# TimoLassmann/kalign

Hardware: AMD Instinct MI355X
Metric: GCUPS (DP cell updates/s) on NxL synthetic MSA (higher is better)
Workload: dtype f32

## Files before the change

kalign_amd/csrc/ka_meetup.h:

```cpp
#pragma once

struct KaLevelOut { int2* items; int* prog; int* nitems; int2* pack16; int2* pack4; int* n16; int* n4; int* nsub; int* rowalloc; int srows;
                    int sub_ok, kind, nres, sub_bytes; };
#define KA_ITEM_SUBTREE 2
#define KA_SUB_MARK 0x7fffffff

__device__ __forceinline__ bool ka_child_is_subtree(const KaLevelOut& o, int rows, int cols)
{
        return o.sub_ok && rows <= KA_SUB_MAXROWS && ka_sub_bytes(o.kind, o.nres, rows, cols) <= o.sub_bytes && cols < 4096;
}

#if KA_TP
#define KA_LONG_COLS 40
#else
#define KA_LONG_COLS 96
#endif
__device__ __forceinline__ bool ka_pass_is_strip(int nrows, int ncols) { return nrows > 32 || (nrows > 2 && ncols >= KA_LONG_COLS); }

__device__ __forceinline__ void ka_emit_pass(const KaLevelOut& o, int slot, int dir, int nrows, int ncols)
{
        if (ka_pass_is_strip(nrows, ncols)) {
                const int ns = ka_strips_of(nrows, o.srows);
                const int base = atomicAdd(o.nitems, ns);
                for (int k = 0; k < ns; ++k) { o.items[base + k] = make_int2(slot, (dir << 16) | k); o.prog[base + k] = 0; }
        } else if (nrows > 8) {
                o.pack16[atomicAdd(o.n16, 1)] = make_int2(slot, dir);
        } else {
                o.pack4[atomicAdd(o.n4, 1)] = make_int2(slot, dir);
        }
}

__device__ __forceinline__ void ka_emit_items(const KaLevelOut& o, int slot, int starta, int enda, int ncols, bool allow_sub = true)
{
        if (allow_sub && ka_child_is_subtree(o, enda - starta, ncols)) {
                const int base = atomicAdd(o.nitems, 1);
                o.items[base] = make_int2(slot, KA_ITEM_SUBTREE << 16); o.prog[base] = 0;
                return;
        }
        const int mid = ((enda - starta) / 2) + starta;
        ka_emit_pass(o, slot, KA_FWD, mid - starta, ncols);
        ka_emit_pass(o, slot, KA_BWD, enda - mid, ncols);
}

__device__ __forceinline__ int ka_level_srows(const TaskShared& S, int level)
{
        if (!S.q1_lvl) return S.srows;
        if (S.split || level > 12) return KA_STRIP_ROWS;
        const int pr = (S.La + (2 << level) - 1) >> (level + 1);
        const long long strips = (long long)(2 << level) * ((pr + KA_STRIP1_ROWS - 1) / KA_STRIP1_ROWS);
        return strips <= 4ll * S.G ? KA_STRIP1_ROWS : KA_STRIP_ROWS;
}

__device__ __forceinline__ KaLevelOut ka_level_out(TaskShared& S, int parity, bool next)
{
        KaLevelOut o;
        o.items = S.items[parity]; o.prog = S.prog[parity];
        o.pack16 = S.pack[parity][0]; o.pack4 = S.pack[parity][1];
        (void)next;
        o.nitems = &S.lctl->lvl[parity].nitems;
        o.n16 = &S.lctl->lvl[parity].npack[0];
        o.n4 = &S.lctl->lvl[parity].npack[1];
        o.nsub = &S.lctl->lvl[parity].nsub;
        o.rowalloc = &S.lctl->lvl[parity].rowalloc;
        o.srows = S.lvl_srows[parity];
        o.sub_ok = S.sub_ok; o.kind = S.kind; o.nres = S.nres_t; o.sub_bytes = S.sub_stride;
        return o;
}

template <int KIND, int GL, bool FLIP = false, bool REC = false, bool MW = false, bool RU = false>
__device__ __forceinline__ void ka_meetup(TaskShared& S, const KaSub* qc, const int k0, const int ncur, KaSub* qnext,
                                          const KaLevelOut& lout, const int wlane, const bool top_level, const int kdig = 0, const int lvl = 0)
{
        static_assert(!MW || GL == 64, "the multi-wave scan works on 64-lane groups");
        const int lane = wlane % GL;
        const int ksub = k0 + wlane / GL;
        const bool in_range = ksub < ncur;
        const KaSub sb = qc[in_range ? ksub : k0];
        const bool rec = REC || S.rec_on;
        const bool valid = in_range && (FLIP || rec || sb.pad != KA_SUB_MARK);
        const bool is_top = top_level && ksub == 0;
        const int startb = sb.startb, endb = sb.endb;
        const int mid = ((sb.enda - sb.starta) / 2) + sb.starta;
        const bool ru = RU && S.reuse_ok != 0;
        const bool f_taken = ru && sb.fsrc >= 0, b_taken = ru && sb.bsrc >= 0;
        const KaState* f = f_taken ? S.sfbuf[(lvl + 1) & 1] + sb.fsrc : S.fbuf + sb.roff;
        const KaState* b = b_taken ? S.sbbuf[(lvl + 1) & 1] + sb.bsrc : S.bbuf + sb.roff;
        const float middle = (float)(endb - startb) / 2.0f + (float)startb;
        const int rrec = mid + 1;
        float g3, g7, g6n, g6f;
        if (KIND == KA_SS) {
                g3 = -S.gpo; g7 = -S.gpo;
                g6n = (startb == 0) ? -S.tgpe : -S.gpe;
                g6f = (endb == S.Lb) ? -S.tgpe : -S.gpe;
        } else {
                const float* R = S.p1 + ((long long)rrec << 6);
                g3 = R[55] * S.p1_mult; g7 = R[55 - 64] * S.p1_mult;
                g6n = (startb == 0) ? R[57] * S.p1_mult : R[56] * S.p1_mult;
                g6f = (endb == S.Lb) ? R[57] * S.p1_mult : R[56] * S.p1_mult;
        }
        Best B = { -KA_F, -KA_F, 0x7fffffff, 0x7fffffff };
        const int mw_wave = MW ? (int)(threadIdx.x >> 6) : 0, mw_nw = MW ? KA_NW : 1;
        for (int i = startb + lane + GL * mw_wave; valid && i <= endb; i += GL * mw_nw) {
                KaState fi = f[i - startb], bi = b[i - startb];
                if (RU) { if (b_taken && i == startb) bi.ga = -KA_F; if (f_taken && i == endb) fi.ga = -KA_F; }
                float sub = fabsf(middle - (float)i);
                sub = sub / 1000.0f;
                const int kb = (i - startb) * 8;
                if (i < endb) {
                        float c2, c5, dummy1, dummy2;
                        col_terms<KIND>(S, i + 1, c2, dummy1, dummy2);
                        col_terms<KIND>(S, i, c5, dummy1, dummy2);
                        best_consider(B, fi.a + bi.a - sub, kb + 0);
                        best_consider(B, fi.a + bi.ga + c2 - sub, kb + 1);
                        best_consider(B, fi.a + bi.gb + g3 - sub, kb + 2);
                        best_consider(B, fi.ga + bi.a + c5 - sub, kb + 3);
                        best_consider(B, fi.gb + bi.gb + g6n - sub, kb + 4);
                        best_consider(B, fi.gb + bi.a + g7 - sub, kb + 5);
                } else {
                        best_consider(B, fi.a + bi.gb + g3 - sub, kb + 2);
                        best_consider(B, fi.gb + bi.gb + g6f - sub, kb + 4);
                }
        }
#pragma unroll
        for (int off = GL / 2; off >= 1; off >>= 1) {
                const float omx = __shfl_xor(B.mx, off, 64);
                const float omx2 = __shfl_xor(B.mx2, off, 64);
                const int okey = __shfl_xor(B.key, off, 64);
                const int okey2 = FLIP ? __shfl_xor(B.key2, off, 64) : 0x7fffffff;
                best_merge(B, omx, omx2, okey, okey2);
        }
        if (MW) {
                if (lane == 0) { S.mw_mx[mw_wave] = B.mx; S.mw_mx2[mw_wave] = B.mx2; S.mw_key[mw_wave] = B.key; }
                __syncthreads();
                if (mw_wave != 0) return;
                B.mx = -KA_F; B.mx2 = -KA_F; B.key = 0x7fffffff; B.key2 = 0x7fffffff;
                for (int w = 0; w < mw_nw; ++w) best_merge(B, S.mw_mx[w], S.mw_mx2[w], S.mw_key[w]);
        }
        const bool leader = (lane == 0) && valid;
        int meet = -1, tr = -1;
        if (leader && B.key != 0x7fffffff) {
                const int ord = B.key & 7;
                meet = startb + (B.key >> 3);
                tr = ord + 1 + (ord >= 3 ? 1 : 0);
        }
        if (leader && is_top) { S.ctl->top_meet = meet; S.ctl->top_tr = tr; S.ctl->top_score = B.mx; }
        if (rec && leader && B.mx2 > -KA_F) {
                const int idx = atomicAdd(&S.ctl->nrec, 1);
                S.mrec[idx] = make_int2(sb.pad, __float_as_int(B.mx - B.mx2));
                if (REC && S.inc) { const KaInc I = ka_inc_view(S); I.win[idx] = sb; I.mx[idx] = make_int2(3 * kdig, S.raw[sb.starta]); }
        }
        if (FLIP && leader) {
                if (B.mx2 > -KA_F) { S.rf.msum += B.mx - B.mx2; S.rf.mcount += 1; }
                if (S.rf.thr > 0.0f && B.key2 != 0x7fffffff && B.mx2 > -KA_F) {
                        const float margin = B.mx - B.mx2;
                        if (margin < S.rf.thr) {
                                if (S.rf.trial > 0 && S.rf.counter % S.rf.stride == S.rf.trial - 1) {
                                        const int ord2 = B.key2 & 7;
                                        meet = startb + (B.key2 >> 3);
                                        tr = ord2 + 1 + (ord2 >= 3 ? 1 : 0);
                                }
                                S.rf.counter += 1;
                        }
                }
        }

        const KaState Z = { 0.0f, -KA_F, -KA_F };
        const KaState GA = { -KA_F, 0.0f, -KA_F };
        const KaState GB = { -KA_F, -KA_F, 0.0f };
        KaSub c1, c2;
        c1.starta = sb.starta; c1.startb = startb; c1.fin = sb.fin;
        c2.enda = sb.enda; c2.endb = endb; c2.bin = sb.bin;
        c1.enda = c1.starta; c1.endb = c1.startb; c1.bin = Z;
        c2.starta = c2.enda; c2.startb = c2.endb; c2.fin = Z;
        c1.pad = rec ? sb.pad + kdig : 0; c2.pad = rec ? sb.pad + 2 * kdig : 0; c1.roff = 0; c2.roff = 0;
        c1.fsrc = -1; c1.bsrc = -1; c2.fsrc = -1; c2.bsrc = -1;
        if (tr > 0) {
                int* path = S.raw;
                switch (tr) {
                case 1:
                        path[mid] = meet; path[mid + 1] = meet + 1;
                        c1.enda = mid - 1; c1.endb = meet - 1; c1.bin = Z;
                        c2.starta = mid + 1; c2.startb = meet + 1; c2.fin = Z;
                        break;
                case 2:
                        path[mid] = meet;
                        c1.enda = mid - 1; c1.endb = meet - 1; c1.bin = Z;
                        c2.starta = mid; c2.startb = meet + 1; c2.fin = GA;
                        break;
                case 3:
                        path[mid] = meet;
                        c1.enda = mid - 1; c1.endb = meet - 1; c1.bin = Z;
                        c2.starta = mid + 1; c2.startb = meet; c2.fin = GB;
                        break;
                case 5:
                        path[mid + 1] = meet + 1;
                        c1.enda = mid; c1.endb = meet - 1; c1.bin = GA;
                        c2.starta = mid + 1; c2.startb = meet + 1; c2.fin = Z;
                        break;
                case 6:
                        c1.enda = mid - 1; c1.endb = meet; c1.bin = GB;
                        c2.starta = mid + 1; c2.startb = meet; c2.fin = GB;
                        break;
                default:
                        path[mid + 1] = meet + 1;
                        c1.enda = mid - 1; c1.endb = meet; c1.bin = GB;
                        c2.starta = mid + 1; c2.startb = meet + 1; c2.fin = Z;
                        break;
                }
        }
        const bool v1 = (tr > 0) && c1.starta < c1.enda && c1.startb < c1.endb;
        const bool v2 = (tr > 0) && c2.starta < c2.enda && c2.startb < c2.endb;
        int need[5] = {0, 0, 0, 0, 0};
        int pr[4], pc[4];
        {
                const int m1 = ((c1.enda - c1.starta) / 2) + c1.starta, m2 = ((c2.enda - c2.starta) / 2) + c2.starta;
                pr[0] = m1 - c1.starta; pr[1] = c1.enda - m1; pr[2] = m2 - c2.starta; pr[3] = c2.enda - m2;
                pc[0] = pc[1] = c1.endb - c1.startb; pc[2] = pc[3] = c2.endb - c2.startb;
        }
        if (v1) { need[0] += 1; need[1] += c1.endb - c1.startb + 1; }
        if (v2) { need[0] += 1; need[1] += c2.endb - c2.startb + 1; }
        const bool st1 = !FLIP && !rec && v1 && ka_child_is_subtree(lout, c1.enda - c1.starta, c1.endb - c1.startb);
        const bool st2 = !FLIP && !rec && v2 && ka_child_is_subtree(lout, c2.enda - c2.starta, c2.endb - c2.startb);
        if (st1) need[2] += 1;
        if (st2) need[2] += 1;
        bool take_f1 = false, take_b2 = false;
        if (RU && ru && !FLIP && !rec) {
                const int nfp = mid - sb.starta, nbp = sb.enda - mid, pcols = endb - startb;
                const int rs_f = (nfp - 1) / 2, rs_b = nbp / 2;
                take_f1 = v1 && !st1 && !f_taken && rs_f >= 1 && ka_pass_is_strip(nfp, pcols) && pr[0] == rs_f;
                take_b2 = v2 && !st2 && !b_taken && rs_b >= 1 && ka_pass_is_strip(nbp, pcols) && pr[3] == rs_b;
                if (take_f1) c1.fsrc = sb.roff;
                if (take_b2) c2.bsrc = sb.roff + (c2.startb - startb);
        }
#pragma unroll
        for (int x = 0; x < 4; ++x) {
                if (!((x < 2) ? v1 : v2) || ((x < 2) ? st1 : st2)) continue;
                if (RU && ((x == 0 && take_f1) || (x == 3 && take_b2))) continue;
                if (ka_pass_is_strip(pr[x], pc[x])) need[2] += ka_strips_of(pr[x], lout.srows);
                else if (pr[x] > 8) need[3] += 1;
                else need[4] += 1;
        }
        float marg = 0.0f;
        int mc = 0;
        if (leader && B.mx2 > -KA_F) { marg = B.mx - B.mx2; mc = 1; }
        int off[5], tot[5];
#pragma unroll
        for (int x = 0; x < 5; ++x) {
                int sc = need[x];
#pragma unroll
                for (int d = 1; d < 64; d <<= 1) { const int y = __shfl_up(sc, d, 64); if (wlane >= d) sc += y; }
                tot[x] = __shfl(sc, 63, 64);
                off[x] = sc - need[x];
        }
        double msum_w = (double)marg;
        int mcnt_w = mc;
#pragma unroll
        for (int d = 32; d >= 1; d >>= 1) { msum_w += __shfl_xor(msum_w, d, 64); mcnt_w += __shfl_xor(mcnt_w, d, 64); }
        int base[5] = {0, 0, 0, 0, 0};
        if (wlane == 0) {
                if (tot[0]) base[0] = atomicAdd(lout.nsub, tot[0]);
                if (tot[1]) base[1] = atomicAdd(lout.rowalloc, tot[1]);
                if (tot[2]) base[2] = atomicAdd(lout.nitems, tot[2]);
                if (tot[3]) base[3] = atomicAdd(lout.n16, tot[3]);
                if (tot[4]) base[4] = atomicAdd(lout.n4, tot[4]);
                if (mcnt_w) { atomicAdd(&S.lctl->msum, msum_w); atomicAdd(&S.lctl->mcount, mcnt_w); }
        }
#pragma unroll
        for (int x = 0; x < 5; ++x) base[x] = __shfl(base[x], 0, 64) + off[x];
        if (!leader || tr < 0) return;
        int slot = base[0], row = base[1], ip = base[2], p16 = base[3], p4 = base[4];
#pragma unroll
        for (int ch = 0; ch < 2; ++ch) {
                KaSub& cs = ch ? c2 : c1;
                if (!(ch ? v2 : v1)) continue;
                cs.roff = row; row += cs.endb - cs.startb + 1;
                if (ch ? st2 : st1) cs.pad = KA_SUB_MARK;
                qnext[slot] = cs;
                if (ch ? st2 : st1) {
                        lout.items[ip] = make_int2(slot, KA_ITEM_SUBTREE << 16); lout.prog[ip] = 0; ++ip; ++slot;
                        continue;
                }
#pragma unroll
                for (int x = 0; x < 2; ++x) {
                        const int nrows = pr[2 * ch + x], ncols = pc[2 * ch + x], dir = x ? KA_BWD : KA_FWD;
                        if (RU && ((ch == 0 && x == 0 && take_f1) || (ch == 1 && x == 1 && take_b2))) continue;
                        if (ka_pass_is_strip(nrows, ncols)) {
                                const int ns = ka_strips_of(nrows, lout.srows);
                                for (int k = 0; k < ns; ++k) { lout.items[ip + k] = make_int2(slot, (dir << 16) | k); lout.prog[ip + k] = 0; }
                                ip += ns;
                        } else if (nrows > 8) {
                                lout.pack16[p16++] = make_int2(slot, dir);
                        } else {
                                lout.pack4[p4++] = make_int2(slot, dir);
                        }
                }
                ++slot;
        }
}
```

kalign_amd/csrc/ka_path.h:

```cpp
#pragma once

__device__ void ka_code_path(TaskShared& S, int* lds)
{
        const int tid = threadIdx.x;
        const int len_a = S.len_a, len_b = S.len_b;
        const int* raw = S.raw;
        if (S.swapped) {
                int* r2 = S.raw2;
                for (int i = tid; i < len_a + 2; i += KA_NT) r2[i] = -1;
                __syncthreads();
                for (int i = 1 + tid; i <= len_b; i += KA_NT) { const int c = S.raw[i]; if (c != -1) r2[c] = i; }
                __syncthreads();
                raw = r2;
        }
        int* o = S.coded;
        int* tot_ops = lds;
        int* tot_b = lds + KA_NT;
        int* zmin = lds + 2 * KA_NT;
        int* zmax = zmin + 1;
        const int per = (len_a + KA_NT - 1) / KA_NT;
        const int lo = 1 + tid * per, hi = min(len_a + 1, lo + per);
        auto row_gaps = [&](int i, int cur, int prev) -> int {
                if (cur == -1) return 0;
                if (i == 1) return cur - 1;
                return (cur - 1 != prev && prev != -1) ? (cur - prev - 1) : 0;
        };
        int nops = 0, nb = 0;
        for (int i = lo; i < hi; ++i) {
                const int cur = raw[i], prev = (i > 1) ? raw[i - 1] : -1;
                const int g = row_gaps(i, cur, prev);
                nops += g + 1;
                nb += g + (cur != -1 ? 1 : 0);
        }
        const int lane_ = tid & 63, wave_ = tid >> 6;
        int sc_ops = nops, sc_b = nb;
#pragma unroll
        for (int d = 1; d < 64; d <<= 1) {
                const int y1 = __shfl_up(sc_ops, d, 64), y2 = __shfl_up(sc_b, d, 64);
                if (lane_ >= d) { sc_ops += y1; sc_b += y2; }
        }
        if (lane_ == 63) { tot_ops[wave_] = sc_ops; tot_b[wave_] = sc_b; }
        if (tid == 0) { *zmin = 0x7fffffff; *zmax = 0; }
        __syncthreads();
        int off = sc_ops - nops, offb = sc_b - nb, all_ops = 0, total_b = 0;
        for (int k = 0; k < KA_NW; ++k) {
                const int a = tot_ops[k], b2 = tot_b[k];
                if (k < wave_) { off += a; offb += b2; }
                all_ops += a; total_b += b2;
        }
        const int last = raw[len_a];
        const int tail = (last != -1 && last < len_b) ? (len_b - last) : 0;
        const int alnlen = all_ops + tail;
        int my_zmin = 0x7fffffff, my_zmax = 0;
        int j = 1 + off, rb = 1 + offb;
        for (int i = lo; i < hi; ++i) {
                const int cur = raw[i], prev = (i > 1) ? raw[i - 1] : -1;
                const int g = row_gaps(i, cur, prev);
                for (int k = 0; k < g; ++k) { o[j] = 1; S.srcA[j] = -1; S.srcB[j] = rb++; ++j; }
                if (cur == -1) { o[j] = 2; S.srcA[j] = i; S.srcB[j] = -1; }
                else { o[j] = 0; S.srcA[j] = i; S.srcB[j] = rb++; my_zmin = min(my_zmin, j); my_zmax = max(my_zmax, j); }
                ++j;
        }
        if (my_zmax > 0) { atomicMin(zmin, my_zmin); atomicMax(zmax, my_zmax); }
        for (int k = tid; k < tail; k += KA_NT) { o[1 + all_ops + k] = 1; S.srcA[1 + all_ops + k] = -1; S.srcB[1 + all_ops + k] = 1 + total_b + k; }
        if (tid == 0) { o[0] = alnlen; o[alnlen + 1] = 3; S.ctl->alnlen = alnlen; }
        __syncthreads();
        const int z1 = *zmin, z2 = *zmax;
        for (int c = 1 + tid; c <= alnlen; c += KA_NT) if (c < z1 || c > z2) o[c] |= 32;
        __syncthreads();
}

__device__ void ka_code_path_refine(TaskShared& S, int* lds)
{
        const int tid = threadIdx.x;
        const int len_a = S.len_a, len_b = S.len_b;
        const int* raw = S.raw;
        if (S.swapped) {
                int* r2 = S.raw2;
                for (int i = tid; i < len_a + 2; i += KA_NT) r2[i] = -1;
                __syncthreads();
                for (int i = 1 + tid; i <= len_b; i += KA_NT) { const int c = S.raw[i]; if (c != -1) r2[c] = i; }
                __syncthreads();
                raw = r2;
        }
        int* o = S.coded;
        int* tot_ops = lds;
        int* tot_b = lds + KA_NT;
        int* tot_m = lds + 2 * KA_NT;
        int* zmin = lds + 3 * KA_NT;
        int* zmax = zmin + 1;
        const int per = (len_a + KA_NT - 1) / KA_NT;
        const int lo = 1 + tid * per, hi = min(len_a + 1, lo + per);
        int mymax = 0;
        for (int i = lo; i < hi; ++i) mymax = max(mymax, raw[i]);
        const int lane_ = tid & 63, wave_ = tid >> 6;
        int sc_m = mymax;
#pragma unroll
        for (int d = 1; d < 64; d <<= 1) { const int y = __shfl_up(sc_m, d, 64); if (lane_ >= d) sc_m = max(sc_m, y); }
        if (lane_ == 63) tot_m[wave_] = sc_m;
        if (tid == 0) { *zmin = 0x7fffffff; *zmax = 0; }
        __syncthreads();
        int blast = __shfl_up(sc_m, 1, 64);
        if (lane_ == 0) blast = 0;
        for (int k = 0; k < wave_; ++k) blast = max(blast, tot_m[k]);
        blast = max(blast, 0);
        int nops = 0, nb = 0;
        {
                int bl = blast;
                for (int i = lo; i < hi; ++i) {
                        const int cur = raw[i];
                        if (cur == -1) { nops += 1; }
                        else { const int gpre = max(cur - bl - 1, 0); nops += gpre + 1; nb += gpre + 1; bl = cur; }
                }
        }
        int sc_ops = nops, sc_b = nb;
#pragma unroll
        for (int d = 1; d < 64; d <<= 1) {
                const int y1 = __shfl_up(sc_ops, d, 64), y2 = __shfl_up(sc_b, d, 64);
                if (lane_ >= d) { sc_ops += y1; sc_b += y2; }
        }
        if (lane_ == 63) { tot_ops[wave_] = sc_ops; tot_b[wave_] = sc_b; }
        __syncthreads();
        int off = sc_ops - nops, offb = sc_b - nb, all_ops = 0, total_b = 0, all_max = 0;
        for (int k = 0; k < KA_NW; ++k) {
                const int a = tot_ops[k], b2 = tot_b[k];
                if (k < wave_) { off += a; offb += b2; }
                all_ops += a; total_b += b2; all_max = max(all_max, tot_m[k]);
        }
        all_max = max(all_max, 0);
        const int tail = len_b - all_max;
        const int alnlen = all_ops + tail;
        int my_zmin = 0x7fffffff, my_zmax = 0;
        {
                int j = 1 + off, rb = 1 + offb, bl = blast;
                for (int i = lo; i < hi; ++i) {
                        const int cur = raw[i];
                        if (cur == -1) { o[j] = 2; S.srcA[j] = i; S.srcB[j] = -1; ++j; }
                        else {
                                const int gpre = max(cur - bl - 1, 0);
                                for (int k = 0; k < gpre; ++k) { o[j] = 1; S.srcA[j] = -1; S.srcB[j] = rb++; ++j; }
                                o[j] = 0; S.srcA[j] = i; S.srcB[j] = rb++;
                                my_zmin = min(my_zmin, j); my_zmax = max(my_zmax, j);
                                ++j; bl = cur;
                        }
                }
        }
        if (my_zmax > 0) { atomicMin(zmin, my_zmin); atomicMax(zmax, my_zmax); }
        for (int k = tid; k < tail; k += KA_NT) { o[1 + all_ops + k] = 1; S.srcA[1 + all_ops + k] = -1; S.srcB[1 + all_ops + k] = 1 + total_b + k; }
        if (tid == 0) { o[0] = alnlen; o[alnlen + 1] = 3; S.ctl->alnlen = alnlen; }
        __syncthreads();
        const int z1 = *zmin, z2 = *zmax;
        for (int c = 1 + tid; c <= alnlen; c += KA_NT) {
                const int t = o[c] & 3;
                int v = t;
                if (t != 0) {
                        if (c >= 2) {
                                const int tp = o[c - 1] & 3;
                                if (tp == 0) v |= 4; else if (tp == t) v |= 8;
                        }
                        if (c <= alnlen - 1 && (o[c + 1] & 3) == 0) { if (v & 8) v += 8; else v |= 16; }
                }
                if (c < z1 || c > z2) v |= 32;
                S.raw2[c] = v;
        }
        __syncthreads();
        for (int c = 1 + tid; c <= alnlen; c += KA_NT) o[c] = S.raw2[c];
        __syncthreads();
}
```

kalign_amd/csrc/ka_task.h:

```cpp
#pragma once

#ifndef KA_RU_TREE
#define KA_RU_TREE 0
#endif
#define KA_LDS_DBG 1400
#define KA_LDS_TSS 1408
#define KA_LDS_WAVES 4096
static_assert(KA_LDS_TSS + 23 * KA_T_STRIDE * 4 <= KA_LDS_WAVES - KA_LDS_HO_BACK, "score table overlaps the hand-over control words");
static_assert(KA_LDS_TSS + 23 * KA_T_STRIDE * 4 <= KA_LDS_WAVES, "score table overlaps the wave regions");
#define KA_LDS_TOTAL (KA_LDS_WAVES + KA_WAVES * KA_WAVE_LDS)
#define KA_HALF_BLOCK 256
#define KA_LDS_HALF (KA_LDS_WAVES + (KA_HALF_BLOCK / 64) * KA_WAVE_LDS)
#define KA_LEAN_SCRATCH(nt_) ((((2 * (nt_) + 16) * 4) + 15) & ~15)
#define KA_LDS_PAIR (KA_LDS_WAVES + KA_LEAN_SCRATCH(KA_PAIR_BLOCK) + (KA_PAIR_BLOCK / 64) * KA_WAVE_LDS_LEAN)
#define KA_LDS_LEAN (KA_LDS_WAVES + KA_LEAN_SCRATCH(KA_LEAN_BLOCK) + (KA_LEAN_BLOCK / 64) * KA_WAVE_LDS_LEAN)
static_assert(sizeof(TaskShared) <= KA_LDS_DBG, "TaskShared outgrew its LDS slot");
static_assert(KA_LDS_WAVES % 16 == 0, "wave regions must be 16-B aligned");

__device__ void ka_build_tss(float* tss, const float* subm, float soff)
{
        for (int x = threadIdx.x; x < 23 * KA_T_STRIDE; x += KA_NT) {
                const int a = x / KA_T_STRIDE, b = x % KA_T_STRIDE;
                tss[x] = (b < 23) ? (subm[23 * a + b] - soff) : 0.0f;
        }
// ... 162 lines not shown
                        __builtin_amdgcn_fence(__ATOMIC_ACQUIRE, "agent");
                        tk0 = __builtin_amdgcn_s_memtime();
                }
                const int len_a = __hip_atomic_load(&D.node_len[T.a], __ATOMIC_RELAXED, __HIP_MEMORY_SCOPE_AGENT);
                const int len_b = __hip_atomic_load(&D.node_len[T.b], __ATOMIC_RELAXED, __HIP_MEMORY_SCOPE_AGENT);
                S.watchdog = D.error; S.trace = D.trace; S.dbgskip = D.flags >> 16;
                S.prof = (D.timing && T.is_root) ? (D.timing + 8ll * (D.numseq - 1) + 48) : nullptr;
                S.len_a = len_a; S.len_b = len_b;
                S.profa = D.prof_arena + __hip_atomic_load(&D.node_prof[T.a], __ATOMIC_RELAXED, __HIP_MEMORY_SCOPE_AGENT);
                S.profb = D.prof_arena + __hip_atomic_load(&D.node_prof[T.b], __ATOMIC_RELAXED, __HIP_MEMORY_SCOPE_AGENT);
                S.subm = D.subm;
                S.gpo = T.gpo; S.gpe = T.gpe; S.tgpe = T.tgpe; S.soff = T.soff;
                S.s1 = nullptr; S.s2 = nullptr; S.p1 = nullptr; S.p2 = nullptr;
                S.sp_open = 0.0f; S.sp_ext = 0.0f; S.sp_text = 0.0f;
                int swapped = 0, kind;
                if (T.nsip_a == 1 && T.nsip_b == 1) {
                        kind = KA_SS;
                        if (len_a < len_b) { S.s1 = D.codes + D.seq_off[T.a]; S.s2 = D.codes + D.seq_off[T.b]; }
                        else { swapped = 1; S.s1 = D.codes + D.seq_off[T.b]; S.s2 = D.codes + D.seq_off[T.a]; }
                } else if (T.nsip_a == 1) {
                        kind = KA_SP; swapped = 1;
                        S.s2 = D.codes + D.seq_off[T.a]; S.p1 = S.profb;
                        S.sp_open = T.gpo * (float)T.nsip_b; S.sp_ext = T.gpe * (float)T.nsip_b; S.sp_text = T.tgpe * (float)T.nsip_b;
                } else if (T.nsip_b == 1) {
                        kind = KA_SP;
                        S.s2 = D.codes + D.seq_off[T.b]; S.p1 = S.profa;
                        S.sp_open = T.gpo * (float)T.nsip_a; S.sp_ext = T.gpe * (float)T.nsip_a; S.sp_text = T.tgpe * (float)T.nsip_a;
                } else {
                        kind = KA_PP;
                        if (len_a < len_b) { S.p1 = S.profa; S.p2 = S.profb; }
                        else { swapped = 1; S.p1 = S.profb; S.p2 = S.profa; }
                }
                S.kind = kind; S.swapped = swapped;
                S.p1_mult = swapped ? (float)T.nsip_a : (float)T.nsip_b;
                S.p2_mult = swapped ? (float)T.nsip_b : (float)T.nsip_a;
                S.La = swapped ? len_b : len_a;
                S.Lb = swapped ? len_a : len_b;
                int g_eff = (S.La >= 1536) ? 8 : ((S.La >= 1152) ? 6 : ((S.La >= 768) ? 4 : ((S.La >= 320) ? 2 : 1)));
                int srows = KA_STRIP_ROWS;
                int q1_lvl = 0;
                if (Q1 && D.q1_mode == 4) {
                        if (D.hw_mode && kind == KA_PP) {
                                const int s1 = ka_strips_of(S.La / 2, KA_STRIP1_ROWS) + ka_strips_of(S.La - S.La / 2, KA_STRIP1_ROWS);
                                q1_lvl = 1;
                                g_eff = max(g_eff, min(g_launch, (s1 + 3) / 4));
                        }
                } else if (Q1 && D.q1_mode) {
                        const int s1 = ka_strips_of(S.La / 2, KA_STRIP1_ROWS) + ka_strips_of(S.La - S.La / 2, KA_STRIP1_ROWS);
                        const int g1 = (s1 + 3) / 4;
                        if (g1 <= g_launch || (D.q1_mode >= 2 && (s1 + 7) / 8 <= g_launch) || D.q1_mode >= 3) { srows = KA_STRIP1_ROWS; g_eff = g1; }
                }
                S.q1_lvl = q1_lvl;
                S.lvl_srows[0] = srows; S.lvl_srows[1] = srows;
                S.ho_ok = (Q1 && NB == 0 && D.ho_mode && kind == KA_PP) ? 1 : 0;
                S.hw_ok = (Q1 && D.hw_mode && kind == KA_PP) ? D.hw_mode : 0;
                if (Q1 && kind == KA_PP) {
                        const int s2 = ka_strips_of(S.La / 2, srows) + ka_strips_of(S.La - S.La / 2, srows);
                        g_eff = (S.ho_ok && D.ho_mode >= 2) ? max((s2 + 3) / 4, 1) : max(g_eff, (s2 + 3) / 4);
                        if (S.hw_ok && !q1_lvl) {
                                int need = s2;
                                for (int l = 1; l < 5; ++l) {
                                        const int rows = (S.La + (2 << l) - 1) >> (l + 1);
                                        if (rows < 2 * srows) break;
                                        need = max(need, (2 << l) * ka_strips_of(rows, srows));
                                }
                                g_eff = max(g_eff, min(g_launch, (need + 3) / 4));
                        }
                }
                if (Q1 && D.per_target > 0 && kind == KA_PP) {
                        const int s2 = ka_strips_of(S.La / 2, srows) + ka_strips_of(S.La - S.La / 2, srows);
                        g_eff = max((s2 + D.per_target - 1) / D.per_target, 1);
                }
                S.carried = (NB && D.cons_K > 0 && ka_votes_carried(D, T)) ? 1 : 0;
                if (NB && D.cons_K > 0 && T.nsip_a + T.nsip_b >= 128) {
                        const int mem = max(T.nsip_a, T.nsip_b);
                        g_eff = max(g_eff, 2 * D.cons_K * (mem >= 1536 ? 3 : (mem >= 384 ? 2 : 1)));
                }
                if (g_eff > g_launch) g_eff = g_launch;
                S.srows = srows;
                S.rec_on = (D.flags & KA_FLAG_EXACT_CONFIDENCE) ? 1 : 0;
                S.sub_ok = (D.sub_mode && !S.rec_on) ? D.sub_mode : 0;
                S.reuse_ok = (KA_RU_TREE && !Q1 && D.reuse && g_eff == 1 && !S.rec_on) ? 1 : 0;
                S.nres_t = (D.nres <= 5) ? 5 : ((D.nres <= 20) ? 20 : 23);
                S.sub_stride = LEAN ? KA_WAVE_LDS_LEAN : KA_WAVE_LDS;
                S.sub_base = LEAN ? (lds_waves + KA_LEAN_SCRATCH(KA_NT)) : lds_waves;
                S.mw_ok = D.mw_mode;
                S.sub_tm = (D.timing && (D.prof_task >= 0 ? task == D.prof_task : T.is_root)) ? 1 : 0;
                for (int x = 0; x < 7; ++x) S.sub_t[x] = 0;
                S.G = g_eff; S.member = member; S.bar_phase = 0;
                S.Gw = g_eff; S.member_w = member; S.split = 0;
                S.ctl = (g_eff == 1) ? &S.ctl_lds : (D.ctl + task);
                S.lctl = S.ctl;
                if (g_eff == 1) { S.ctl_lds.fail = 0; S.ctl_lds.bar = 0; S.ctl_lds.nrec = 0; S.ctl_lds.vote_conf = 0; S.ctl_lds.vote_types = 0; }
                s_dbg = nullptr;
                if (member == 0) {
                        const long long need = ka_scratch_bytes(len_a, len_b, NB ? D.cons_maxlen : 0, g_eff, false, (D.flags & KA_FLAG_EXACT_CONFIDENCE) != 0, NB ? NB : KA_NB, NB > KA_NB ? D.cons_K : -1);
                        const unsigned long long so = atomicAdd(&D.counters[1], (unsigned long long)need);
                        if ((long long)so + need > D.scratch_cap) { S.ctl->fail = 1; atomicExch(D.error, 2); }
                        if (__hip_atomic_load(D.error, __ATOMIC_RELAXED, __HIP_MEMORY_SCOPE_AGENT) != 0) S.ctl->fail = 1;
                        S.ctl->scratch_off = (long long)so;
                        if (D.flags & KA_FLAG_DEBUG_ROWS) {
                                const unsigned long long nd = 6ull * (unsigned long long)(S.Lb + 1);
                                const unsigned long long d0 = atomicAdd(&D.counters[3], nd);
                                if ((long long)(d0 + nd) <= D.dbg_cap) { s_dbg = D.dbg_arena + d0; D.dbg_off[task] = (long long)d0; }
                                else { D.dbg_off[task] = -1; atomicExch(D.error, 4); }
                        }
                }
        }
        __syncthreads();
        if (S.member >= S.G) return 2;
        ka_cluster_sync(S);
        if (S.ctl->fail) return 1;
        if (tid == 0) ka_carve(S, D.scratch + S.ctl->scratch_off, S.len_a, S.len_b, NB ? D.cons_maxlen : 0, false, S.rec_on != 0, NB ? NB : KA_NB, NB > KA_NB ? D.cons_K : -1);

        ka_build_tss(tss, D.subm, T.soff);
        __syncthreads();
        const bool leaf_syn = !(D.usw > 0.0f) && !(D.flags & KA_FLAG_LEAF_PROFILES);
        if (S.member == 0 && !leaf_syn) {
                if (T.nsip_a == 1) ka_make_leaf_profile(S.profa, S.len_a, D.codes + D.seq_off[T.a], T.gpo, T.gpe, T.tgpe, tss);
                if (T.nsip_b == 1) ka_make_leaf_profile(S.profb, S.len_b, D.codes + D.seq_off[T.b], T.gpo, T.gpe, T.tgpe, tss);
        }
        if (NB) {
                __syncthreads();
                if (S.carried) { if (S.member == 0) ka_cons_from_tables(S, D, T); }
                else ka_cons_votes<LEAN, (NB ? NB : KA_NB)>(S, D, T, lds_waves, LEAN ? 0 : (long long)KA_NW * KA_WAVE_LDS);
                ka_cluster_sync(S);
                if (S.member == 0) ka_cons_entries<(NB ? NB : KA_NB)>(S, D);
        }
        ka_cluster_sync(S);
        tk1 = __builtin_amdgcn_s_memtime();
        if (tid == 0 && blockIdx.x == 0) KA_CRUMB(D.trace, 4, 2);

        if (LEAN || S.kind == KA_SS) ka_hirschberg<KA_SS, 23, NB, false, Q1, false, false, KA_RU_TREE && !Q1>(S, s_dbg, lds_waves, tss, D.trace);
        else if (S.kind == KA_SP) ka_hirschberg<KA_SP, 23, NB, false, Q1, false, false, KA_RU_TREE && !Q1>(S, s_dbg, lds_waves, tss, D.trace);
        else if (D.nres <= 5) ka_hirschberg<KA_PP, 5, NB, false, Q1, Q1 && NB == 0, Q1, KA_RU_TREE && !Q1>(S, s_dbg, lds_waves, tss, D.trace);
#ifdef KA_FAKE_NRES
        else if (D.nres <= 20) ka_hirschberg<KA_PP, KA_FAKE_NRES, NB, false, Q1, Q1 && NB == 0, Q1, KA_RU_TREE && !Q1>(S, s_dbg, lds_waves, tss, D.trace);
#else
        else if (D.nres <= 20) ka_hirschberg<KA_PP, 20, NB, false, Q1, Q1 && NB == 0, Q1, KA_RU_TREE && !Q1>(S, s_dbg, lds_waves, tss, D.trace);
#endif
        else ka_hirschberg<KA_PP, 23, NB, false, Q1, Q1 && NB == 0, Q1, KA_RU_TREE && !Q1>(S, s_dbg, lds_waves, tss, D.trace);
        __syncthreads();
        bool conf_exact = false;
        if (S.rec_on && S.member == 0 && S.n_levels < KA_REC_DEPTH) {
                if (tid == 0) { S.mlog = nullptr; S.mlog_cap = 0; }
                __syncthreads();
                const int cap = (int)min((long long)KA_REC_SORT_CAP, (LEAN ? (long long)KA_NW * KA_WAVE_LDS_LEAN + KA_LEAN_SCRATCH(KA_NT) : (long long)KA_NW * KA_WAVE_LDS) / 8);
                conf_exact = ka_margins_in_order(S, lds_waves, cap);
        }
        tk2 = __builtin_amdgcn_s_memtime();
        if (tid == 0 && blockIdx.x == 0) KA_CRUMB(D.trace, 4, 3);
#undef s_dbg

        if (S.member == 0) {
                ka_code_path(S, (int*)lds_waves);
                if (tid == 0) {
                        const int alnlen = S.ctl->alnlen;
                        const unsigned long long pn = (unsigned long long)alnlen + 2;
                        const unsigned long long po = atomicAdd(&D.counters[2], pn);
                        if ((long long)(po + pn) > D.path_cap) { S.ctl->fail = 1; atomicExch(D.error, 3); }
                        S.ctl->path_off = (long long)po;
                        S.ctl->newp_off = -1;
                        D.node_len[T.c] = alnlen;
                        if (!T.is_root) {
                                const bool votes = NB && D.cons_K > 0 && S.carried;
                                const unsigned long long fn = pn * 64ull + (votes ? 5ull * (unsigned long long)D.cons_K * pn : 0ull);
                                const unsigned long long fo = atomicAdd(&D.counters[0], fn);
                                if ((long long)(fo + fn) > D.prof_cap) { S.ctl->fail = 1; atomicExch(D.error, 1); }
                                else { S.ctl->newp_off = (long long)fo; D.node_prof[T.c] = (long long)fo; if (votes) D.node_vote[T.c] = (long long)(fo + pn * 64ull); }
                        }
                        ka_task_rec r;
                        r.a = T.a; r.b = T.b; r.c = T.c;
                        r.len_a = S.len_a; r.len_b = S.len_b; r.nsip_a = T.nsip_a; r.nsip_b = T.nsip_b;
                        r.plen = alnlen; r.kind = S.kind; r.swapped = S.swapped;
                        r.meet = S.ctl->top_meet; r.transition = S.ctl->top_tr;
                        r.path_off = (int)po;
                        r.gap_scale = T.gap_scale; r.subm_off = T.soff;
                        r.score = S.ctl->top_score;
                        r.confidence = (S.ctl->mcount > 0) ? (float)S.ctl->msum / (float)S.ctl->mcount : 0.0f;
                        if (conf_exact) r.confidence = (S.rf.mcount > 0) ? S.rf.msum / (float)S.rf.mcount : 0.0f;
                        r.prof_hash = 0; r.fhash = 0; r.bhash = 0;
                        D.recs[task] = r;
                }
        }
        ka_cluster_sync(S);
        tk3 = __builtin_amdgcn_s_memtime();
        if (S.ctl->fail) return 1;

        if (tid == 0) {
                S.path_dst = D.path_arena + S.ctl->path_off;
                S.newp = (S.ctl->newp_off >= 0) ? (D.prof_arena + S.ctl->newp_off) : nullptr;
        }
        __syncthreads();
        const int alnlen = S.ctl->alnlen;
        if (S.member == 0) for (int i = tid; i < alnlen + 2; i += KA_NT) S.path_dst[i] = S.coded[i];
        if (S.newp) ka_update_profile(S, D, T, alnlen, leaf_syn ? tss : nullptr);
        if ((NB && !T.is_root) || (D.flags & KA_FLAG_DEVICE_GAPS)) ka_update_colof(S, D, T, alnlen);
        if (NB && D.cons_K > 0 && S.carried && S.newp) ka_votes_merge(S, D, T, alnlen, (int*)(S.newp + ((long long)alnlen + 2) * 64));
        if (D.timing && S.member == 0) {
                __syncthreads();
                if (tid == 0) {
                        long long* tm = D.timing + 8ll * task;
                        tm[0] = tk1 - tk0; tm[1] = tk2 - tk1; tm[2] = tk3 - tk2; tm[3] = __builtin_amdgcn_s_memtime() - tk3;
                        tm[4] = S.t_pass; tm[5] = S.t_meet; tm[6] = S.n_levels | (S.G << 8) | (g_launch << 16); tm[7] = (long long)S.La * S.Lb;
                        if (D.prof_task >= 0 ? task == D.prof_task : T.is_root) {
                                long long* lv = D.timing + 8ll * (D.numseq - 1);
                                for (int l = 0; l < 16; ++l) {
                                        lv[3 * l] = l < S.n_levels ? S.lvl_n[l] : 0;
                                        lv[3 * l + 1] = l < S.n_levels ? S.lvl_pass[l] : 0;
                                        lv[3 * l + 2] = l < S.n_levels ? S.lvl_meet[l] : 0;
                                }
                                if (S.n_levels <= 13) for (int x = 0; x < 7; ++x) lv[41 + x] = (long long)S.sub_t[x];
                        }
                }
        }
        return 0;
}

template <int NB>
__device__ __forceinline__ void ka_task_body_refine(const KaTreeDev& D, const int task, const int member, const int G)
{
        extern __shared__ __attribute__((aligned(16))) char ka_smem[];
        TaskShared& S = *(TaskShared*)ka_smem;
        float* tss = (float*)(ka_smem + KA_LDS_TSS);
        char* lds_waves = ka_smem + KA_LDS_WAVES;
        const KaTaskDesc T = D.tasks[task];
        const int tid = threadIdx.x;
        long long tq[7] = {0, 0, 0, 0, 0, 0, 0};
        long long tlast = __builtin_amdgcn_s_memtime();
        auto lap = [&](int k) { const long long now = __builtin_amdgcn_s_memtime(); tq[k] += now - tlast; tlast = now; };
        if (tid == 0) {
                const int len_a = D.node_len[T.a], len_b = D.node_len[T.b];
                S.watchdog = D.error; S.trace = D.trace; S.dbgskip = ((D.wdfs & 1) ? 0 : 1) | ((D.wdfs & 8) ? 0 : 2); S.prof = nullptr;
                S.len_a = len_a; S.len_b = len_b;
                S.profa = D.prof_arena + D.node_prof[T.a];
                S.profb = D.prof_arena + D.node_prof[T.b];
                S.subm = D.subm;
                S.gpo = T.gpo; S.gpe = T.gpe; S.tgpe = T.tgpe; S.soff = T.soff;
                S.s1 = nullptr; S.s2 = nullptr; S.p1 = nullptr; S.p2 = nullptr;
                S.sp_open = 0.0f; S.sp_ext = 0.0f; S.sp_text = 0.0f;
                int swapped = 0, kind;
                if (T.nsip_a == 1 && T.nsip_b == 1) {
                        kind = KA_SS;
                        if (len_a < len_b) { S.s1 = D.codes + D.seq_off[T.a]; S.s2 = D.codes + D.seq_off[T.b]; }
                        else { swapped = 1; S.s1 = D.codes + D.seq_off[T.b]; S.s2 = D.codes + D.seq_off[T.a]; }
                } else if (T.nsip_a == 1) {
                        kind = KA_SP; swapped = 1;
                        S.s2 = D.codes + D.seq_off[T.a]; S.p1 = S.profb;
                        S.sp_open = T.gpo * (float)T.nsip_b; S.sp_ext = T.gpe * (float)T.nsip_b; S.sp_text = T.tgpe * (float)T.nsip_b;
                } else if (T.nsip_b == 1) {
                        kind = KA_SP;
                        S.s2 = D.codes + D.seq_off[T.b]; S.p1 = S.profa;
                        S.sp_open = T.gpo * (float)T.nsip_a; S.sp_ext = T.gpe * (float)T.nsip_a; S.sp_text = T.tgpe * (float)T.nsip_a;
                } else {
                        kind = KA_PP;
                        if (len_a < len_b) { S.p1 = S.profa; S.p2 = S.profb; }
                        else { swapped = 1; S.p1 = S.profb; S.p2 = S.profa; }
                }
                S.kind = kind; S.swapped = swapped;
                S.p1_mult = swapped ? (float)T.nsip_a : (float)T.nsip_b;
                S.p2_mult = swapped ? (float)T.nsip_b : (float)T.nsip_a;
                S.La = swapped ? len_b : len_a;
                S.Lb = swapped ? len_a : len_b;
                S.G = 1; S.member = 0; S.bar_phase = 0; S.Gw = 1; S.member_w = 0; S.split = 0; S.srows = KA_STRIP_ROWS; S.q1_lvl = 0; S.lvl_srows[0] = KA_STRIP_ROWS; S.lvl_srows[1] = KA_STRIP_ROWS;
                S.reuse_ok = 0;
                S.sub_ok = 0; S.rec_on = 0; S.nres_t = 23; S.sub_stride = 0; S.sub_base = nullptr; S.sub_tm = 0; S.mw_ok = 0;
                S.ctl = &S.ctl_lds; S.lctl = S.ctl;
                S.ctl_lds.fail = 0; S.ctl_lds.bar = 0; S.ctl_lds.vote_conf = 0; S.ctl_lds.vote_types = 0;
                S.carried = (NB && D.cons_K > 0 && ka_votes_carried(D, T)) ? 1 : 0;
                const long long need = ka_scratch_bytes(len_a, len_b, NB ? D.cons_maxlen : 0, 1, true, false, NB ? NB : KA_NB, NB > KA_NB ? D.cons_K : -1);
                const unsigned long long so = atomicAdd(&D.counters[1], (unsigned long long)need);
                if ((long long)so + need > D.scratch_cap) { S.ctl->fail = 1; atomicExch(D.error, 2); }
                if (__hip_atomic_load(D.error, __ATOMIC_RELAXED, __HIP_MEMORY_SCOPE_AGENT) != 0) S.ctl->fail = 1;
                S.ctl->scratch_off = (long long)so;
                if (!S.ctl->fail) ka_carve(S, D.scratch + so, len_a, len_b, NB ? D.cons_maxlen : 0, true, false, NB ? NB : KA_NB, NB > KA_NB ? D.cons_K : -1);
        }
        __syncthreads();
        if (S.ctl->fail) return;

        ka_build_tss(tss, D.subm, T.soff);
        __syncthreads();
        if (T.nsip_a == 1) ka_make_leaf_profile(S.profa, S.len_a, D.codes + D.seq_off[T.a], T.gpo, T.gpe, T.tgpe, tss);
        if (T.nsip_b == 1) ka_make_leaf_profile(S.profb, S.len_b, D.codes + D.seq_off[T.b], T.gpo, T.gpe, T.tgpe, tss);
        if (NB) {
                __syncthreads();
                if (S.carried) ka_cons_from_tables(S, D, T);
                else ka_cons_votes<false, (NB ? NB : KA_NB)>(S, D, T, lds_waves, (long long)KA_NW * KA_WAVE_LDS);
                __syncthreads();
                ka_cons_entries<(NB ? NB : KA_NB)>(S, D);
        }
        const bool inline_mode = D.refine_mode == 3;
        const bool refine_it = D.refine_mode == 1 || inline_mode || (D.refine_mode == 2 && T.refine != 0);
        int n_trials = inline_mode ? max(D.refine_trials, 1) : refine_it ? 5 : 1;
        const bool adaptive_it = D.refine_adaptive && refine_it && !inline_mode;
        lap(0);
        if (refine_it) ka_sp_build(S, D, T);
        __syncthreads();
        lap(1);

        float best_sp = -KA_F, avg_margin = 0.0f, best_msum = 0.0f;
        int best_mcount = 0, best_k = 0;
        int top_meet0 = -1, top_tr0 = -1;
        bool inc_ok = false, inc_listed = false;
        float top_score0 = 0.0f;
        const int Gt = (refine_it && G > 1) ? G : 1;
        if (member >= Gt) return;
        for (int k = 0; k < n_trials; ++k) {
                if (k > 0 && (k - 1) % Gt != member) continue;
                if (tid == 0) {
                        S.rf.thr = (k == 0) ? 0.0f : avg_margin; S.rf.trial = k; S.rf.stride = max(n_trials - 1, 1);
                        S.mlog = (adaptive_it && k == 0) ? (float*)S.raw2 : nullptr;
                        S.mlog_cap = min(max(min(S.len_a, S.len_b) + 1, 64), S.len_a + S.len_b + 8);
                        S.adapt_trials = 0;
                }
                __syncthreads();
                bool done = false;
                if (k == 0 && (D.wdfs & 2) && S.La < (1 << 17)) {
                        inc_ok = false;
                        if (tid == 0) S.ctl->nrec = 0;
                        __syncthreads();
                        if (S.kind == KA_SS) ka_hirschberg<KA_SS, 23, NB, true>(S, nullptr, lds_waves, tss, D.trace);
                        else if (S.kind == KA_SP) ka_hirschberg<KA_SP, 23, NB, true>(S, nullptr, lds_waves, tss, D.trace);
                        else if (D.nres <= 5) ka_hirschberg<KA_PP, 5, NB, true>(S, nullptr, lds_waves, tss, D.trace);
                        else ka_hirschberg<KA_PP, 23, NB, true>(S, nullptr, lds_waves, tss, D.trace);
                        __syncthreads();
                        done = ka_margins_in_order(S, lds_waves);
                        inc_ok = done && (n_trials > 1 || adaptive_it) && (D.wdfs & 4) && S.inc != nullptr;
                        if (inc_ok) ka_inc_build(S, lds_waves);
                }
                if (k > 0 && inc_ok) {
                        if (!inc_listed) { ka_inc_uncertain(S, avg_margin); inc_listed = true; }
                        if (S.kind == KA_SS) ka_trial_incremental<KA_SS, 23, NB>(S, lds_waves, tss);
                        else if (S.kind == KA_SP) ka_trial_incremental<KA_SP, 23, NB>(S, lds_waves, tss);
                        else if (D.nres <= 5) ka_trial_incremental<KA_PP, 5, NB>(S, lds_waves, tss);
                        else ka_trial_incremental<KA_PP, 23, NB>(S, lds_waves, tss);
                        done = true;
                }
                if (!done) {
                        if (S.kind == KA_SS) ka_hirschberg_dfs<KA_SS, 23, NB>(S, lds_waves, tss, k == 0);
                        else if (S.kind == KA_SP) ka_hirschberg_dfs<KA_SP, 23, NB>(S, lds_waves, tss, k == 0);
                        else if (D.nres <= 5) ka_hirschberg_dfs<KA_PP, 5, NB>(S, lds_waves, tss, k == 0);
                        else ka_hirschberg_dfs<KA_PP, 23, NB>(S, lds_waves, tss, k == 0);
                }
                __syncthreads();
                lap(2);
                if (k == 0 && adaptive_it) {
                        const int mc = S.rf.mcount;
                        if (mc > 0) {
// ... 259 lines not shown
```

Measured before the change: 55.98.

## Batch global loads in meet scan, path coding, and path copy; parallelize counter atomics

The meet-point scan now issues KA_MEET_BATCH clamped global loads up front through address_space(1) pointers, and for profile-profile alignment reads the p2 gap terms directly, so several loads are in flight at once. The level-counter atomics are spread across lanes 0-4 with writelane instead of being issued serially by lane 0. ka_code_path prefetches raw path entries in batches of 8 and returns alnlen. The task epilogue sets path_dst and newp from thread 0 and skips a syncthreads for member 0. The path copy is batched four-wide. This raises register pressure and depends on the KaCtl::Lvl counter layout, which a static_assert checks.

After: 55.97, median of 3. About the same (-0.0%).

```diff
diff --git a/kalign_amd/csrc/ka_meetup.h b/kalign_amd/csrc/ka_meetup.h
--- a/kalign_amd/csrc/ka_meetup.h
+++ b/kalign_amd/csrc/ka_meetup.h
@@ -3,6 +3,7 @@
 struct KaLevelOut { int2* items; int* prog; int* nitems; int2* pack16; int2* pack4; int* n16; int* n4; int* nsub; int* rowalloc; int srows;
                     int sub_ok, kind, nres, sub_bytes; };
 #define KA_ITEM_SUBTREE 2
+#define KA_MEET_BATCH 4
 #define KA_SUB_MARK 0x7fffffff
 
 __device__ __forceinline__ bool ka_child_is_subtree(const KaLevelOut& o, int rows, int cols)
@@ -87,38 +88,58 @@
         const KaState* b = b_taken ? S.sbbuf[(lvl + 1) & 1] + sb.bsrc : S.bbuf + sb.roff;
         const float middle = (float)(endb - startb) / 2.0f + (float)startb;
         const int rrec = mid + 1;
+        typedef const __attribute__((address_space(1))) float* ka_gfc;
+        const ka_gfc gf = (ka_gfc)(const float*)f, gb = (ka_gfc)(const float*)b;
         float g3, g7, g6n, g6f;
         if (KIND == KA_SS) {
                 g3 = -S.gpo; g7 = -S.gpo;
                 g6n = (startb == 0) ? -S.tgpe : -S.gpe;
                 g6f = (endb == S.Lb) ? -S.tgpe : -S.gpe;
         } else {
-                const float* R = S.p1 + ((long long)rrec << 6);
-                g3 = R[55] * S.p1_mult; g7 = R[55 - 64] * S.p1_mult;
-                g6n = (startb == 0) ? R[57] * S.p1_mult : R[56] * S.p1_mult;
-                g6f = (endb == S.Lb) ? R[57] * S.p1_mult : R[56] * S.p1_mult;
+                const ka_gfc R = (ka_gfc)(S.p1 + ((long long)rrec << 6));
+                const float r55 = R[55], r55m = R[55 - 64], r56 = R[56], r57 = R[57];
+                g3 = r55 * S.p1_mult; g7 = r55m * S.p1_mult;
+                g6n = (startb == 0) ? r57 * S.p1_mult : r56 * S.p1_mult;
+                g6f = (endb == S.Lb) ? r57 * S.p1_mult : r56 * S.p1_mult;
         }
         Best B = { -KA_F, -KA_F, 0x7fffffff, 0x7fffffff };
         const int mw_wave = MW ? (int)(threadIdx.x >> 6) : 0, mw_nw = MW ? KA_NW : 1;
-        for (int i = startb + lane + GL * mw_wave; valid && i <= endb; i += GL * mw_nw) {
-                KaState fi = f[i - startb], bi = b[i - startb];
-                if (RU) { if (b_taken && i == startb) bi.ga = -KA_F; if (f_taken && i == endb) fi.ga = -KA_F; }
-                float sub = fabsf(middle - (float)i);
-                sub = sub / 1000.0f;
-                const int kb = (i - startb) * 8;
-                if (i < endb) {
-                        float c2, c5, dummy1, dummy2;
-                        col_terms<KIND>(S, i + 1, c2, dummy1, dummy2);
-                        col_terms<KIND>(S, i, c5, dummy1, dummy2);
-                        best_consider(B, fi.a + bi.a - sub, kb + 0);
-                        best_consider(B, fi.a + bi.ga + c2 - sub, kb + 1);
-                        best_consider(B, fi.a + bi.gb + g3 - sub, kb + 2);
-                        best_consider(B, fi.ga + bi.a + c5 - sub, kb + 3);
-                        best_consider(B, fi.gb + bi.gb + g6n - sub, kb + 4);
-                        best_consider(B, fi.gb + bi.a + g7 - sub, kb + 5);
-                } else {
-                        best_consider(B, fi.a + bi.gb + g3 - sub, kb + 2);
-                        best_consider(B, fi.gb + bi.gb + g6f - sub, kb + 4);
+        const int cstep = GL * mw_nw;
+        const ka_gfc gp2 = (KIND == KA_PP) ? (ka_gfc)S.p2 : nullptr;
+        const float p2m = (KIND == KA_PP) ? S.p2_mult : 0.0f;
+        for (int i0 = startb + lane + GL * mw_wave; valid && i0 <= endb; i0 += KA_MEET_BATCH * cstep) {
+                float fa[KA_MEET_BATCH], fga[KA_MEET_BATCH], fgb[KA_MEET_BATCH], ba[KA_MEET_BATCH], bga[KA_MEET_BATCH], bgb[KA_MEET_BATCH];
+                float o2[KA_MEET_BATCH], o5[KA_MEET_BATCH];
+#pragma unroll
+                for (int u = 0; u < KA_MEET_BATCH; ++u) {
+                        const int ic = min(i0 + u * cstep, endb), x = 3 * (ic - startb);
+                        fa[u] = gf[x]; fga[u] = gf[x + 1]; fgb[u] = gf[x + 2];
+                        ba[u] = gb[x]; bga[u] = gb[x + 1]; bgb[u] = gb[x + 2];
+                        if (KIND == KA_PP) { o5[u] = gp2[((long long)ic << 6) + 55]; o2[u] = gp2[((long long)min(ic + 1, endb) << 6) + 55]; }
+                }
+#pragma unroll
+                for (int u = 0; u < KA_MEET_BATCH; ++u) {
+                        const int i = i0 + u * cstep;
+                        if (i > endb) break;
+                        KaState fi = { fa[u], fga[u], fgb[u] }, bi = { ba[u], bga[u], bgb[u] };
+                        if (RU) { if (b_taken && i == startb) bi.ga = -KA_F; if (f_taken && i == endb) fi.ga = -KA_F; }
+                        float sub = fabsf(middle - (float)i);
+                        sub = sub / 1000.0f;
+                        const int kb = (i - startb) * 8;
+                        if (i < endb) {
+                                float c2, c5, dummy1, dummy2;
+                                if (KIND == KA_PP) { c2 = o2[u] * p2m; c5 = o5[u] * p2m; }
+                                else { col_terms<KIND>(S, i + 1, c2, dummy1, dummy2); col_terms<KIND>(S, i, c5, dummy1, dummy2); }
+                                best_consider(B, fi.a + bi.a - sub, kb + 0);
+                                best_consider(B, fi.a + bi.ga + c2 - sub, kb + 1);
+                                best_consider(B, fi.a + bi.gb + g3 - sub, kb + 2);
+                                best_consider(B, fi.ga + bi.a + c5 - sub, kb + 3);
+                                best_consider(B, fi.gb + bi.gb + g6n - sub, kb + 4);
+                                best_consider(B, fi.gb + bi.a + g7 - sub, kb + 5);
+                        } else {
+                                best_consider(B, fi.a + bi.gb + g3 - sub, kb + 2);
+                                best_consider(B, fi.gb + bi.gb + g6f - sub, kb + 4);
+                        }
                 }
         }
 #pragma unroll
@@ -256,17 +277,21 @@
         int mcnt_w = mc;
 #pragma unroll
         for (int d = 32; d >= 1; d >>= 1) { msum_w += __shfl_xor(msum_w, d, 64); mcnt_w += __shfl_xor(mcnt_w, d, 64); }
-        int base[5] = {0, 0, 0, 0, 0};
-        if (wlane == 0) {
-                if (tot[0]) base[0] = atomicAdd(lout.nsub, tot[0]);
-                if (tot[1]) base[1] = atomicAdd(lout.rowalloc, tot[1]);
-                if (tot[2]) base[2] = atomicAdd(lout.nitems, tot[2]);
-                if (tot[3]) base[3] = atomicAdd(lout.n16, tot[3]);
-                if (tot[4]) base[4] = atomicAdd(lout.n4, tot[4]);
-                if (mcnt_w) { atomicAdd(&S.lctl->msum, msum_w); atomicAdd(&S.lctl->mcount, mcnt_w); }
-        }
-#pragma unroll
-        for (int x = 0; x < 5; ++x) base[x] = __shfl(base[x], 0, 64) + off[x];
+        int base[5];
+        {
+                static_assert(offsetof(KaCtl::Lvl, nsub) == 0 && offsetof(KaCtl::Lvl, rowalloc) == 4 && offsetof(KaCtl::Lvl, nitems) == 8
+                              && offsetof(KaCtl::Lvl, npack) == 16, "the level's counters, as lanes 0 - 4 address them");
+                int my_tot = 0;
+#define KA_TOT_TO_LANE(x_) asm("v_writelane_b32 %0, %1, " #x_ : "+v"(my_tot) : "s"(__builtin_amdgcn_readfirstlane(tot[x_])))
+                KA_TOT_TO_LANE(0); KA_TOT_TO_LANE(1); KA_TOT_TO_LANE(2); KA_TOT_TO_LANE(3); KA_TOT_TO_LANE(4);
+#undef KA_TOT_TO_LANE
+                int* const my_ctr = lout.nsub + (wlane + (wlane >= 3 ? 1 : 0));
+                int my_base = 0;
+                if (wlane < 5 && my_tot) my_base = atomicAdd(my_ctr, my_tot);
+                if (wlane == 0 && mcnt_w) { atomicAdd(&S.lctl->msum, msum_w); atomicAdd(&S.lctl->mcount, mcnt_w); }
+#pragma unroll
+                for (int x = 0; x < 5; ++x) base[x] = __shfl(my_base, x, 64) + off[x];
+        }
         if (!leader || tr < 0) return;
         int slot = base[0], row = base[1], ip = base[2], p16 = base[3], p4 = base[4];
 #pragma unroll
diff --git a/kalign_amd/csrc/ka_path.h b/kalign_amd/csrc/ka_path.h
--- a/kalign_amd/csrc/ka_path.h
+++ b/kalign_amd/csrc/ka_path.h
@@ -1,6 +1,7 @@
 #pragma once
 
-__device__ void ka_code_path(TaskShared& S, int* lds)
+#define KA_CODE_BATCH 8
+__device__ int ka_code_path(TaskShared& S, int* lds)
 {
         const int tid = threadIdx.x;
         const int len_a = S.len_a, len_b = S.len_b;
@@ -20,17 +21,39 @@
         int* zmax = zmin + 1;
         const int per = (len_a + KA_NT - 1) / KA_NT;
         const int lo = 1 + tid * per, hi = min(len_a + 1, lo + per);
-        auto row_gaps = [&](int i, int cur, int prev) -> int {
+        auto row_gaps = [](int i, int cur, int prev) -> int {
                 if (cur == -1) return 0;
                 if (i == 1) return cur - 1;
                 return (cur - 1 != prev && prev != -1) ? (cur - prev - 1) : 0;
         };
+        typedef const __attribute__((address_space(1))) int* ka_gic;
+        const ka_gic graw = (ka_gic)raw;
+        int first[KA_CODE_BATCH];
+        const int before = (lo > 1) ? graw[min(lo - 1, len_a)] : -1;
+#pragma unroll
+        for (int u = 0; u < KA_CODE_BATCH; ++u) first[u] = graw[min(lo + u, len_a)];
+        const int last = graw[len_a];
         int nops = 0, nb = 0;
-        for (int i = lo; i < hi; ++i) {
-                const int cur = raw[i], prev = (i > 1) ? raw[i - 1] : -1;
-                const int g = row_gaps(i, cur, prev);
-                nops += g + 1;
-                nb += g + (cur != -1 ? 1 : 0);
+        {
+                int prev = before;
+                for (int i0 = lo; i0 < hi; i0 += KA_CODE_BATCH) {
+                        int c[KA_CODE_BATCH];
+#pragma unroll
+                        for (int u = 0; u < KA_CODE_BATCH; ++u) c[u] = first[u];
+                        if (i0 != lo) {
+#pragma unroll
+                                for (int u = 0; u < KA_CODE_BATCH; ++u) c[u] = graw[min(i0 + u, len_a)];
+                        }
+#pragma unroll
+                        for (int u = 0; u < KA_CODE_BATCH; ++u) {
+                                if (i0 + u < hi) {
+                                        const int g = row_gaps(i0 + u, c[u], prev);
+                                        nops += g + 1;
+                                        nb += g + (c[u] != -1 ? 1 : 0);
+                                        prev = c[u];
+                                }
+                        }
+                }
         }
         const int lane_ = tid & 63, wave_ = tid >> 6;
         int sc_ops = nops, sc_b = nb;
@@ -48,26 +71,44 @@
                 if (k < wave_) { off += a; offb += b2; }
                 all_ops += a; total_b += b2;
         }
-        const int last = raw[len_a];
         const int tail = (last != -1 && last < len_b) ? (len_b - last) : 0;
         const int alnlen = all_ops + tail;
         int my_zmin = 0x7fffffff, my_zmax = 0;
         int j = 1 + off, rb = 1 + offb;
-        for (int i = lo; i < hi; ++i) {
-                const int cur = raw[i], prev = (i > 1) ? raw[i - 1] : -1;
-                const int g = row_gaps(i, cur, prev);
-                for (int k = 0; k < g; ++k) { o[j] = 1; S.srcA[j] = -1; S.srcB[j] = rb++; ++j; }
-                if (cur == -1) { o[j] = 2; S.srcA[j] = i; S.srcB[j] = -1; }
-                else { o[j] = 0; S.srcA[j] = i; S.srcB[j] = rb++; my_zmin = min(my_zmin, j); my_zmax = max(my_zmax, j); }
-                ++j;
+        int* const srcA = S.srcA;
+        int* const srcB = S.srcB;
+        {
+                int prev = before;
+                for (int i0 = lo; i0 < hi; i0 += KA_CODE_BATCH) {
+                        int c[KA_CODE_BATCH];
+#pragma unroll
+                        for (int u = 0; u < KA_CODE_BATCH; ++u) c[u] = first[u];
+                        if (i0 != lo) {
+#pragma unroll
+                                for (int u = 0; u < KA_CODE_BATCH; ++u) c[u] = graw[min(i0 + u, len_a)];
+                        }
+#pragma unroll
+                        for (int u = 0; u < KA_CODE_BATCH; ++u) {
+                                if (i0 + u < hi) {
+                                        const int i = i0 + u, cur = c[u];
+                                        const int g = row_gaps(i, cur, prev);
+                                        for (int k = 0; k < g; ++k) { o[j] = 1; srcA[j] = -1; srcB[j] = rb++; ++j; }
+                                        if (cur == -1) { o[j] = 2; srcA[j] = i; srcB[j] = -1; }
+                                        else { o[j] = 0; srcA[j] = i; srcB[j] = rb++; my_zmin = min(my_zmin, j); my_zmax = max(my_zmax, j); }
+                                        ++j;
+                                        prev = cur;
+                                }
+                        }
+                }
         }
         if (my_zmax > 0) { atomicMin(zmin, my_zmin); atomicMax(zmax, my_zmax); }
-        for (int k = tid; k < tail; k += KA_NT) { o[1 + all_ops + k] = 1; S.srcA[1 + all_ops + k] = -1; S.srcB[1 + all_ops + k] = 1 + total_b + k; }
+        for (int k = tid; k < tail; k += KA_NT) { o[1 + all_ops + k] = 1; srcA[1 + all_ops + k] = -1; srcB[1 + all_ops + k] = 1 + total_b + k; }
         if (tid == 0) { o[0] = alnlen; o[alnlen + 1] = 3; S.ctl->alnlen = alnlen; }
         __syncthreads();
         const int z1 = *zmin, z2 = *zmax;
         for (int c = 1 + tid; c <= alnlen; c += KA_NT) if (c < z1 || c > z2) o[c] |= 32;
         __syncthreads();
+        return alnlen;
 }
 
 __device__ void ka_code_path_refine(TaskShared& S, int* lds)
diff --git a/kalign_amd/csrc/ka_task.h b/kalign_amd/csrc/ka_task.h
--- a/kalign_amd/csrc/ka_task.h
+++ b/kalign_amd/csrc/ka_task.h
@@ -338,22 +338,27 @@
         if (tid == 0 && blockIdx.x == 0) KA_CRUMB(D.trace, 4, 3);
 #undef s_dbg
 
+        int alnlen = 0;
         if (S.member == 0) {
-                ka_code_path(S, (int*)lds_waves);
+                alnlen = ka_code_path(S, (int*)lds_waves);
                 if (tid == 0) {
-                        const int alnlen = S.ctl->alnlen;
                         const unsigned long long pn = (unsigned long long)alnlen + 2;
+                        const bool votes = NB && D.cons_K > 0 && S.carried;
+                        const unsigned long long fn = pn * 64ull + (votes ? 5ull * (unsigned long long)D.cons_K * pn : 0ull);
                         const unsigned long long po = atomicAdd(&D.counters[2], pn);
+                        const unsigned long long fo = T.is_root ? 0ull : atomicAdd(&D.counters[0], fn);
                         if ((long long)(po + pn) > D.path_cap) { S.ctl->fail = 1; atomicExch(D.error, 3); }
                         S.ctl->path_off = (long long)po;
                         S.ctl->newp_off = -1;
+                        S.path_dst = D.path_arena + (long long)po;
+                        S.newp = nullptr;
                         D.node_len[T.c] = alnlen;
                         if (!T.is_root) {
-                                const bool votes = NB && D.cons_K > 0 && S.carried;
-                                const unsigned long long fn = pn * 64ull + (votes ? 5ull * (unsigned long long)D.cons_K * pn : 0ull);
-                                const unsigned long long fo = atomicAdd(&D.counters[0], fn);
                                 if ((long long)(fo + fn) > D.prof_cap) { S.ctl->fail = 1; atomicExch(D.error, 1); }
-                                else { S.ctl->newp_off = (long long)fo; D.node_prof[T.c] = (long long)fo; if (votes) D.node_vote[T.c] = (long long)(fo + pn * 64ull); }
+                                else {
+                                        S.ctl->newp_off = (long long)fo; S.newp = D.prof_arena + (long long)fo;
+                                        D.node_prof[T.c] = (long long)fo; if (votes) D.node_vote[T.c] = (long long)(fo + pn * 64ull);
+                                }
                         }
                         ka_task_rec r;
                         r.a = T.a; r.b = T.b; r.c = T.c;
@@ -373,13 +378,26 @@
         tk3 = __builtin_amdgcn_s_memtime();
         if (S.ctl->fail) return 1;
 
-        if (tid == 0) {
-                S.path_dst = D.path_arena + S.ctl->path_off;
-                S.newp = (S.ctl->newp_off >= 0) ? (D.prof_arena + S.ctl->newp_off) : nullptr;
-        }
-        __syncthreads();
-        const int alnlen = S.ctl->alnlen;
-        if (S.member == 0) for (int i = tid; i < alnlen + 2; i += KA_NT) S.path_dst[i] = S.coded[i];
+        if (S.member != 0) {
+                if (tid == 0) {
+                        S.path_dst = D.path_arena + S.ctl->path_off;
+                        S.newp = (S.ctl->newp_off >= 0) ? (D.prof_arena + S.ctl->newp_off) : nullptr;
+                }
+                __syncthreads();
+                alnlen = S.ctl->alnlen;
+        }
+        if (S.member == 0) {
+                typedef const __attribute__((address_space(1))) int* ka_gic;
+                const ka_gic gc = (ka_gic)S.coded;
+                int* const pd = S.path_dst;
+                for (int i0 = tid; i0 < alnlen + 2; i0 += 4 * KA_NT) {
+                        int v[4];
+#pragma unroll
+                        for (int u = 0; u < 4; ++u) v[u] = gc[min(i0 + u * KA_NT, alnlen + 1)];
+#pragma unroll
+                        for (int u = 0; u < 4; ++u) if (i0 + u * KA_NT < alnlen + 2) pd[i0 + u * KA_NT] = v[u];
+                }
+        }
         if (S.newp) ka_update_profile(S, D, T, alnlen, leaf_syn ? tss : nullptr);
         if ((NB && !T.is_root) || (D.flags & KA_FLAG_DEVICE_GAPS)) ka_update_colof(S, D, T, alnlen);
         if (NB && D.cons_K > 0 && S.carried && S.newp) ka_votes_merge(S, D, T, alnlen, (int*)(S.newp + ((long long)alnlen + 2) * 64));
```
